# edantec/MPC_benchmark

Hardware: AMD Instinct MI355X
Metric: mpc_solves_per_sec (higher is better)
Workload: dtype f64

## Files before the change

### mpc_benchmark_amd/csrc/legs.h

```cpp
#pragma once
#include "mfma_blocks.h"
#include "solver_kernels.h"

#define LEG_BARRIER() asm volatile("s_waitcnt lgkmcnt(0)\n\ts_barrier" ::: "memory")

#define LEG_LAUNDER() do { asm volatile("" : "+v"(tid), "+v"(lane)); wv = __builtin_amdgcn_readfirstlane(tid >> 6); } while (0)

#define LK_THREADS 512
#define LK_U 20
#define LK_PT 13
#define LK_TILES 5

struct LkLds {
  int np, mp, nzp, lda, ldp, ldm, nb, nbm;
  int AB, PR, TM, ZN, vec, total_bytes;
  unsigned mg_nzp, mg_np, mg_mp;
};
static inline constexpr LkLds make_lk_lds(int n, int m) {
  LkLds s{};
  s.np = (n + 15) & ~15; s.mp = (m + 15) & ~15; s.nzp = s.np + s.mp; s.lda = s.nzp + 1; s.ldp = s.np + 1; s.ldm = s.mp + 1;
  s.nb = s.np / 16; s.nbm = s.mp / 16;
  s.mg_nzp = magic_div(s.nzp); s.mg_np = magic_div(s.np); s.mg_mp = magic_div(s.mp);
  int o = 0;
  auto take = [&](int cnt) { int r = o; o += (cnt + 1) & ~1; return r; };
  const int pr = s.np * s.ldp > s.mp * s.np + s.mp * s.ldm ? s.np * s.ldp : s.mp * s.np + s.mp * s.ldm;
  s.AB = take(s.np * s.lda); s.PR = take(pr); s.TM = take(6 * s.nzp + 6 * s.np + 40); s.ZN = take(16 * s.ldm); s.vec = take(s.mp + 3 * s.np + 80 + 8);
  s.total_bytes = o * 8;
  return s;
}

template <int MP, int FN = 0, int FM = 0>
DEV void leg_knot_body(const SolverArgs& a, const LkLds& Srt, const int b, const int kbeg, const int kend, const int prof_b, const int prof_k) {
  constexpr bool FX = FN > 0;
  constexpr LkLds SC_ = FX ? make_lk_lds(FN, FM) : LkLds{};
  LkLds S_ = Srt;
  if constexpr (FX) S_ = SC_;
  const LkLds& S = S_;
  constexpr int NAB = (80 * (80 + MP) + LK_THREADS - 1) / LK_THREADS, NK = (MP * 80 + LK_THREADS - 1) / LK_THREADS;
  constexpr int NMU = (MP * MP + LK_THREADS - 1) / LK_THREADS, NZN = (16 * MP + LK_THREADS - 1) / LK_THREADS;
  const Layout& L = a.L;
  int tid = threadIdx.x, lane = tid & 63;
  constexpr int nthr = LK_THREADS, nw = LK_THREADS / 64;
  int wv = __builtin_amdgcn_readfirstlane(tid >> 6);
  const InstState& st = a.inst[b];
  if (st.done || st.skip_step) return;
  const int n = FX ? FN : L.n, nz = FX ? FN + FM : L.nz, np = S.np, mp = S.mp, nzp = S.nzp, lda = S.lda, ldp = S.ldp, ldm = S.ldm, nb = S.nb, nbm = S.nbm;
  const double mud = st.mu * a.opt.dyn_al_scale;
  extern __shared__ __attribute__((aligned(16))) double sm[];
  double *AB = sm + S.AB, *PR = sm + S.PR, *ZN = sm + S.ZN, *vec = sm + S.vec;
  double *KM = PR, *PT = PR, *U1 = PR, *MU = PR + mp * np;
  double *TMP = sm + S.TM, *PT6 = TMP + 6 * nzp, *c6 = PT6 + 6 * np;
  double *kf = vec, *y0 = vec + mp, *z0 = y0 + np, *t6 = z0 + np, *g6 = t6 + 36, *mxs = g6 + 36;
  int* cnt = (int*)(mxs + np);
  long long tk0_ = clock64();
#define LK_PROF(slot) do { if (a.prof && k == prof_k && b == prof_b && tid == 0) { const long long t1_ = clock64(); a.prof[prof_b * 64 + 32 + (slot)] += (double)(t1_ - tk0_); tk0_ = t1_; } } while (0)

  double pab[NAB], pkm[NK], ptv[LK_PT], pmu[NMU], pzn[NZN], psm = 0.0, pact = 0.0;
  auto request_ab = [&](int k) {
    const double* kn = knot_ptr(a, b, k);
    const double* g = gain_ptr(a, b, k);
    const int m = (int)kn[L.oMISC + MISC_M], c = (int)kn[L.oMISC + MISC_NC];
#pragma unroll
    for (int u = 0; u < NAB; ++u) {
      const int idx = tid + u * nthr, i = qdiv(idx, S.mg_nzp), zp = (idx - qdiv(idx, S.mg_nzp) * nzp);
      const int z = (zp < n) ? zp : ((zp >= np && zp - np < m) ? n + zp - np : -1);
      pab[u] = (idx < np * nzp && i < n && z >= 0) ? kn[L.oAB + (size_t)i * nz + z] : 0.0;
    }
#pragma unroll
    for (int u = 0; u < NK; ++u) {
      const int idx = tid + u * nthr, l = qdiv(idx, S.mg_np), j = (idx - qdiv(idx, S.mg_np) * np);
      pkm[u] = (idx < mp * np && l < m && j < n) ? g[L.oK + l * n + j] : 0.0;
    }
    psm = (tid < mp) ? ((tid < m) ? g[L.ok + tid] : 0.0) : ((tid >= 64 && tid < 100) ? g[L.oT6 + tid - 64] : ((tid >= 128 && tid < 128 + n) ? g[L.omx + tid - 128] : 0.0));
    pact = (tid < c) ? kn[L.oACT + tid] : 0.0;
  };
  auto request_pt = [&](int k) {
    const double* g = gain_ptr(a, b, k);
#pragma unroll
    for (int u = 0; u < LK_PT; ++u) {
      const int idx = tid + u * nthr, i = qdiv(idx, S.mg_np), j = (idx - qdiv(idx, S.mg_np) * np);
      ptv[u] = (idx < np * np && i < n && j < n) ? g[L.oMx + i * n + j] : 0.0;
    }
  };
  auto request_mu = [&](int k) {
    const double* g = gain_ptr(a, b, k);
#pragma unroll
    for (int u = 0; u < NMU; ++u) { const int idx = tid + u * nthr; pmu[u] = (idx < mp * mp) ? g[L.oMu + idx] : 0.0; }
#pragma unroll
    for (int u = 0; u < NZN; ++u) { const int idx = tid + u * nthr; pzn[u] = (idx < 16 * mp) ? g[L.oZnu + idx] : 0.0; }
  };

  request_ab(kbeg);
  request_pt(kbeg);
  if (leg_of_knot(a, kbeg) + 1 < a.nlegs) request_mu(kbeg);
  for (int k = kbeg; k < kend; ++k) {
    const double* kn = knot_ptr(a, b, k);
    double* g = gain_ptr(a, b, k);
    const int m = (int)kn[L.oMISC + MISC_M];
    const bool par = leg_of_knot(a, k) + 1 < a.nlegs;
    const bool more = k + 1 < kend, par_next = more && leg_of_knot(a, k + 1) + 1 < a.nlegs;
    LEG_BARRIER();
    LEG_LAUNDER();
    if (a.prof) tk0_ = clock64();
#pragma unroll
    for (int u = 0; u < NAB; ++u) { const int idx = tid + u * nthr; if (idx < np * nzp) AB[(qdiv(idx, S.mg_nzp)) * lda + (idx - qdiv(idx, S.mg_nzp) * nzp)] = pab[u]; }
#pragma unroll
    for (int u = 0; u < NK; ++u) { const int idx = tid + u * nthr; if (idx < mp * np) KM[idx] = pkm[u]; }
    if (tid < mp) kf[tid] = psm;
    else if (tid >= 64 && tid < 100) t6[tid - 64] = psm;
    else if (tid >= 128 && tid < 128 + np) mxs[tid - 128] = psm;
    int ca = 0;
    if (par) {
      const unsigned long long act = __ballot(pact != 0.0);
      if (lane == 0) cnt[wv] = __popcll(act);
    }
    LEG_BARRIER();
    if (par) for (int w = 0; w < nw; ++w) ca += cnt[w];
    LEG_LAUNDER();
    if (more) request_ab(k + 1);
    LEG_LAUNDER();
    LK_PROF(0);
    for (int t = wv; t < nb * nb; t += nw) {
      const int ri = t / nb, cj = t % nb;
      double* At = AB + (ri * 16) * lda + cj * 16;
      d4_t acc = tile_load(At, lda, lane);
      mma_tile<false>(acc, AB + (ri * 16) * lda + np, lda, 1, KM + cj * 16, np, 1, mp, lane);
      tile_store(At, lda, acc, lane);
    }
    for (int i = wv; i < np; i += nw) {
      double s = (lane < m) ? AB[i * lda + np + lane] * kf[lane] : 0.0;
      s = wave_sum(s);
      if (lane == 0) y0[i] = s + mxs[i];
    }
    if (tid < 36) { const int i = tid / 6, j = tid % 6; double s = 0; for (int l = 0; l < 6; ++l) s += t6[i * 6 + l] * t6[j * 6 + l]; g6[tid] = s; }
    LEG_BARRIER();
    LEG_LAUNDER();
#pragma unroll
    for (int u = 0; u < LK_PT; ++u) { const int idx = tid + u * nthr; if (idx < np * np) PT[(qdiv(idx, S.mg_np)) * ldp + (idx - qdiv(idx, S.mg_np) * np)] = ptv[u]; }
    LEG_BARRIER();
    LEG_LAUNDER();
    if (more) request_pt(k + 1);
    LEG_LAUNDER();
    LK_PROF(1);
    const int nct = par ? nb + nbm : nb;
    d4_t res[LK_TILES];
#pragma unroll
    for (int sidx = 0; sidx < LK_TILES; ++sidx) {
      const int t = wv + sidx * nw;
      res[sidx] = d4_t{0, 0, 0, 0};
      if (t < nb * nct) mma_tile<false>(res[sidx], PT + ((t / nct) * 16) * ldp, ldp, 1, AB + (t % nct) * 16, lda, 1, np, lane);
    }
    for (int i = wv; i < n; i += nw) {
      double s = 0;
      for (int j = lane; j < n; j += 64) s += PT[i * ldp + j] * y0[j];
      s = wave_sum(s);
      if (lane == 0) z0[i] = y0[i] - mud * s;
    }
    LEG_BARRIER();
#pragma unroll
    for (int sidx = 0; sidx < LK_TILES; ++sidx) {
      const int t = wv + sidx * nw;
      if (t < nb * nct) {
        double* At = AB + ((t / nct) * 16) * lda + (t % nct) * 16;
        const int row = lane >> 4, col = lane & 15;
#pragma unroll
        for (int q = 0; q < 4; ++q) At[(row + 4 * q) * lda + col] -= mud * res[sidx][q];
      }
    }
    LEG_BARRIER();
    LK_PROF(2);
    for (int idx = tid; idx < 6 * nzp; idx += nthr) TMP[idx] = AB[(qdiv(idx, S.mg_nzp)) * lda + (idx - qdiv(idx, S.mg_nzp) * nzp)];
    if (par) for (int idx = tid; idx < np * 6; idx += nthr) {
      const int i = idx / 6, j = idx % 6;
      double s = 0;
      for (int l = 0; l < 6; ++l) s += PT[i * ldp + l] * t6[j * 6 + l];
      PT6[idx] = s;
    }
    LEG_BARRIER();
    for (int idx = tid; idx < 6 * nzp; idx += nthr) {
      const int i = qdiv(idx, S.mg_nzp), z = (idx - qdiv(idx, S.mg_nzp) * nzp);
      double s = 0;
      for (int l = 0; l < 6; ++l) s += t6[i * 6 + l] * TMP[l * nzp + z];
      AB[i * lda + z] = s;
    }
    if (par && tid < 36) {
      const int i = tid / 6, j = tid % 6;
      double s = 0;
      for (int l = 0; l < 6; ++l) s += t6[i * 6 + l] * PT6[l * 6 + j];
      c6[tid] = s;
    }
    LEG_BARRIER();
    for (int i = wv; i < n; i += nw)
      for (int j = lane; j < n; j += 64) g[L.oPhi + i * n + j] = AB[i * lda + j];
    for (int i = tid; i < n; i += nthr) {
      double s = z0[i];
      if (i < 6) { s = 0; for (int l = 0; l < 6; ++l) s += t6[i * 6 + l] * z0[l]; }
      g[L.ophi + i] = s;
    }
    LK_PROF(3);
    LEG_LAUNDER();
    if (par) {
#pragma unroll
      for (int u = 0; u < NMU; ++u) { const int idx = tid + u * nthr; if (idx < mp * mp) MU[(qdiv(idx, S.mg_mp)) * ldm + (idx - qdiv(idx, S.mg_mp) * mp)] = pmu[u]; }
#pragma unroll
      for (int u = 0; u < NZN; ++u) { const int idx = tid + u * nthr; if (idx < 16 * mp) ZN[(qdiv(idx, S.mg_mp)) * ldm + (idx - qdiv(idx, S.mg_mp) * mp)] = (qdiv(idx, S.mg_mp) < ca && ca <= 16) ? pzn[u] : 0.0; }
      LEG_BARRIER();
      LEG_LAUNDER();
      if (par_next) request_mu(k + 1);
      LEG_LAUNDER();
      LK_PROF(4);
      d4_t ures[2];
#pragma unroll
      for (int sidx = 0; sidx < 2; ++sidx) {
        const int t = wv + sidx * nw;
        ures[sidx] = d4_t{0, 0, 0, 0};
        if (t < nbm * nb) mma_tile<false>(ures[sidx], MU + ((t / nb) * 16) * ldm, ldm, 1, AB + ((t % nb) * 16) * lda + np, 1, lda, mp, lane);
      }
#ifdef LK_SUBPROF
      LK_PROF(7);
#endif
      if (ca <= 16) {
        for (int cj = wv; cj < nb; cj += nw) {
          d4_t acc = d4_t{0, 0, 0, 0};
          mma_tile<false>(acc, ZN, ldm, 1, AB + (cj * 16) * lda + np, 1, lda, mp, lane);
          const int col = cj * 16 + (lane & 15);
#pragma unroll
          for (int q = 0; q < 4; ++q) { const int row = (lane >> 4) + 4 * q; if (row < ca && col < n) g[L.oKnup + row * n + col] = -acc[q]; }
        }
      } else {
        for (int idx = tid; idx < ca * n; idx += nthr) {
          const int i = idx / n, j = idx % n;
          double s = 0;
          for (int l = 0; l < m; ++l) s += g[L.oZnu + i * mp + l] * AB[j * lda + np + l];
          g[L.oKnup + idx] = -s;
        }
      }
#ifdef LK_SUBPROF
      LK_PROF(8);
#endif
#pragma unroll
      for (int sidx = 0; sidx < 2; ++sidx) {
        const int t = wv + sidx * nw;
        if (t < nbm * nb) {
          const int ri = t / nb, cj = t % nb, col = cj * 16 + (lane & 15);
#pragma unroll
          for (int q = 0; q < 4; ++q) {
            const int row = ri * 16 + (lane >> 4) + 4 * q;
            U1[row * np + col] = ures[sidx][q];
            if (row < m && col < n) g[L.oKu + row * n + col] = -ures[sidx][q];
          }
        }
      }
#ifdef LK_SUBPROF
      LK_PROF(9);
#endif
      LEG_BARRIER();
      LK_PROF(5);
      for (int t = wv; t < nb * nb; t += nw) {
        const int ri = t / nb, cj = t % nb, col = cj * 16 + (lane & 15);
        double ptt[4];
#pragma unroll
        for (int q = 0; q < 4; ++q) {
          const int row = ri * 16 + (lane >> 4) + 4 * q;
          const bool in = row < n && col < n;
          ptt[q] = (in && row >= 6 && col >= 6) ? g[L.oMx + row * n + col] : 0.0;
        }
        d4_t acc = d4_t{0, 0, 0, 0};
        mma_tile<false>(acc, AB + (ri * 16) * lda + np, lda, 1, U1 + cj * 16, np, 1, mp, lane);
#pragma unroll
        for (int q = 0; q < 4; ++q) {
          const int row = ri * 16 + (lane >> 4) + 4 * q;
          if (row < n && col < n) {
            const double tt = (row < 6 && col < 6) ? g6[row * 6 + col] : (row == col ? 1.0 : 0.0);
            const double tp = (row < 6 && col < 6) ? c6[row * 6 + col] : (col < 6 ? PT6[row * 6 + col] : (row < 6 ? PT6[col * 6 + row] : ptt[q]));
            g[L.oGam + row * n + col] = -acc[q] - mud * (tt - mud * tp);
          }
        }
      }
      LK_PROF(6);
    } else if (par_next) request_mu(k + 1);
  }
}

template <int MP, int FN = 0, int FM = 0>
__global__ void __launch_bounds__(LK_THREADS) k_leg_knot(SolverArgs a, LkLds Srt, int chunk, int kmax) {
  const int kbeg = blockIdx.x * chunk, kend = (kbeg + chunk < kmax) ? kbeg + chunk : kmax;
  if (kbeg < kend) leg_knot_body<MP, FN, FM>(a, Srt, blockIdx.y, kbeg, kend, 1, 1);
}

struct LcLds { int np, ldp, nb; int LM, BA, BB, vec, total_bytes; unsigned mg_np, mg_ldp; };
static inline constexpr int lc_ld(int np) { int ld = np; while ((ld & 31) != 16) ++ld; return ld; }
static inline constexpr LcLds make_lc_lds(int n) {
  LcLds s{};
  s.np = (n + 15) & ~15; s.ldp = lc_ld(s.np); s.nb = s.np / 16;
  s.mg_np = magic_div(s.np); s.mg_ldp = magic_div(s.ldp);
  int o = 0;
  auto take = [&](int cnt) { int r = o; o += (cnt + 1) & ~1; return r; };
  s.LM = take(s.np * s.ldp); s.BA = take(s.np * s.ldp); s.BB = take(s.np * s.ldp); s.vec = take(3 * s.np + 16);
  s.total_bytes = o * 8;
  return s;
}
#define LC_TILES 4
#define LC_STILES 2

template <int FN = 0>
DEV void leg_condense_body(const SolverArgs& a, const LcLds& Srt, const int j, const int b) {
  constexpr bool FX = FN > 0;
  constexpr LcLds SC_ = FX ? make_lc_lds(FN) : LcLds{};
  LcLds S_ = Srt;
  if constexpr (FX) S_ = SC_;
  const LcLds& S = S_;
  const Layout& L = a.L;
  constexpr int nthr = LK_THREADS, nw = LK_THREADS / 64;
  int tid = threadIdx.x, lane = tid & 63, wv = __builtin_amdgcn_readfirstlane(tid >> 6);
  const InstState& st = a.inst[b];
  if (st.done || st.skip_step) return;
  const int n = FX ? FN : L.n, np = S.np, ldp = S.ldp, nb = S.nb;
  const int ks = leg_start(a, j), ke = leg_start(a, j + 1) - 1;
  extern __shared__ __attribute__((aligned(16))) double sm[];
  double *LM = sm + S.LM, *BA = sm + S.BA, *BB = sm + S.BB, *sg = sm + S.vec, *phi = sg + np;
  for (int idx = tid; idx < np * ldp; idx += nthr) { const int i = qdiv(idx, S.mg_ldp), c0 = (idx - qdiv(idx, S.mg_ldp) * ldp); LM[idx] = (i == c0 && i < n) ? 1.0 : 0.0; }
  for (int i = tid; i < np; i += nthr) sg[i] = 0.0;
  d4_t sacc[LC_STILES];
  int tri[LC_STILES], tcj[LC_STILES];
#pragma unroll
  for (int sidx = 0; sidx < LC_STILES; ++sidx) {
    sacc[sidx] = d4_t{0, 0, 0, 0};
    int ri = 0, rem = wv + sidx * nw;
    while (rem > ri) { rem -= ri + 1; ++ri; }
    tri[sidx] = ri; tcj[sidx] = rem;
  }
  const int nst = nb * (nb + 1) / 2;
  double pa[LK_PT], pb[LK_PT], pphi;
  auto prefetch = [&](int kk) {
    const double* gk = gain_ptr(a, b, kk);
#pragma unroll
    for (int u = 0; u < LK_PT; ++u) {
      const int idx = tid + u * nthr, i = qdiv(idx, S.mg_np), c0 = (idx - qdiv(idx, S.mg_np) * np);
      const bool ok = idx < np * np && i < n && c0 < n;
      const int src = ok ? i * n + c0 : 0;
      pa[u] = gk[L.oPhi + src] * (ok ? 1.0 : 0.0);
      pb[u] = gk[L.oGam + src] * (ok ? 1.0 : 0.0);
    }
    pphi = gk[L.ophi + (tid < n ? tid : 0)];
  };
  prefetch(ke);
  long long tc0_ = clock64();
#define LC_PROF(slot) do { if (a.prof && j == 0 && b == 2 && tid == 0) { const long long t1_ = clock64(); a.prof[128 + 32 + (slot)] += (double)(t1_ - tc0_); tc0_ = t1_; } } while (0)
  for (int k = ke; k >= ks; --k) {
    LEG_LAUNDER();
#pragma unroll
    for (int u = 0; u < LK_PT; ++u) {
      const int idx = tid + u * nthr;
      if (idx < np * np) { BA[(qdiv(idx, S.mg_np)) * ldp + (idx - qdiv(idx, S.mg_np) * np)] = pa[u]; BB[(qdiv(idx, S.mg_np)) * ldp + (idx - qdiv(idx, S.mg_np) * np)] = pb[u]; }
    }
    if (tid < np) phi[tid] = (tid < n) ? pphi : 0.0;
    LEG_BARRIER();
    LC_PROF(0);
    LEG_LAUNDER();
    if (k > ks) prefetch(k - 1);
    LEG_LAUNDER();
    d4_t lres[LC_TILES], zres[LC_TILES];
#pragma unroll
    for (int sidx = 0; sidx < LC_TILES; ++sidx) {
      const int t = wv + sidx * nw;
      lres[sidx] = d4_t{0, 0, 0, 0}; zres[sidx] = d4_t{0, 0, 0, 0};
      if (t < nb * nb)
        mma_tile_2a(lres[sidx], zres[sidx], BA + (t / nb) * 16, 1, ldp, BB + (t / nb) * 16, 1, ldp, LM + (t % nb) * 16, ldp, 1, np, lane);
    }
    LC_PROF(1);
    {
      const int ts = tid - (nthr - 128);
      if (ts >= 0 && ts < n) {
        double s = 0;
#pragma unroll 16
        for (int l = 0; l < np; ++l) s += LM[l * ldp + ts] * phi[l];
        sg[ts] += s;
      }
    }
    LC_PROF(2);
    LEG_BARRIER();
    LC_PROF(3);
    LEG_LAUNDER();
#pragma unroll
    for (int sidx = 0; sidx < LC_TILES; ++sidx) {
      const int t = wv + sidx * nw;
      if (t < nb * nb) tile_store(BB + ((t / nb) * 16) * ldp + (t % nb) * 16, ldp, zres[sidx], lane);
    }
    LEG_BARRIER();
    LC_PROF(4);
    LEG_LAUNDER();
#pragma unroll
    for (int sidx = 0; sidx < LC_STILES; ++sidx)
      if (wv + sidx * nw < nst) mma_tile<false>(sacc[sidx], LM + tri[sidx] * 16, 1, ldp, BB + tcj[sidx] * 16, ldp, 1, np, lane);
    LC_PROF(5);
    LEG_BARRIER();
    LC_PROF(6);
    LEG_LAUNDER();
    double* gk = gain_ptr(a, b, k);
#pragma unroll
    for (int sidx = 0; sidx < LC_TILES; ++sidx) {
      const int t = wv + sidx * nw;
      if (t < nb * nb) {
        const int ri = t / nb, cj = t % nb, col = cj * 16 + (lane & 15);
        tile_store(LM + (ri * 16) * ldp + cj * 16, ldp, lres[sidx], lane);
#pragma unroll
        for (int q = 0; q < 4; ++q) { const int row = ri * 16 + (lane >> 4) + 4 * q; if (row < n && col < n) gk[L.oLm + row * n + col] = lres[sidx][q]; }
// ... 499 lines not shown
```

### mpc_benchmark_amd/csrc/mpc_hip.hip

```cpp
#include <hip/hip_runtime.h>
#include <mutex>
#include <map>
#include <cmath>
#include <cstdio>
#include <cstdlib>
#include <cstring>
#include <limits>
#include <stdexcept>
#include <string>
#include <utility>
#include <vector>

#include "eval_multibody_host.h"
#include "eval_reuse_kernels.h"
#include "eval_vector.h"
#include "riccati_mfma.h"
#include "closed_loop.h"
#include "legs.h"
#include "legs_tree.h"
#include "pipeline_glue.h"
#include "pipeline_ikid_glue.h"
#include "pipeline_contacts.h"
#include "pipeline_fd_glue.h"
#include "sim_record.h"
// ... 117 lines not shown
  bool spec_rec_valid = false, spec_next_pending = false, spec_next_now = false;
  int cycles_since_run = 0;
  int khead = 0;
  int* d_spec = nullptr;
  double* d_fext = nullptr;
  int only_knot = -1;
  bool appended_changed = false;
  bool appended_any = false;
  bool walk_on = false, walk_force_all = false;
  std::vector<uint8_t> walk_poisoned;
  mpc_walk_config walk{};
  double* d_walk_state = nullptr;
  double *d_walk_cmd = nullptr, *d_poses_cmd = nullptr;
  bool walk_cmd_on = false, poses_cmd_on = false;
  bool poses_on = false;
  mpc_walk_poses_config poses{};
  double *d_poses_state = nullptr, *d_poses_samples = nullptr, *d_poses_x = nullptr;
  size_t poses_x_cap = 0;
  int since_change = 1 << 20;
  bool refine_now = false;
  SimPlant plant;
  std::vector<uint8_t> slot_dirty;
  bool dirty_all = false;
  bool spec_skip_pass = false;
  unsigned long long dirty_now[MPC_DIRTY_WORDS] = {};
  static constexpr int PATCH_RING = 4;
  char* patch_pin[PATCH_RING] = {};
  size_t patch_cap[PATCH_RING] = {};
  hipEvent_t patch_ev[PATCH_RING] = {};
  int patch_next = 0;
  char* d_patch = nullptr;
  size_t d_patch_cap = 0;
  double* h_xnext[2] = {nullptr, nullptr};
  std::vector<double> leg_mu;
  static constexpr int ASYNC_DEPTH = 2;
  InstState* h_status[ASYNC_DEPTH] = {nullptr, nullptr};
  hipEvent_t status_ev[ASYNC_DEPTH] = {nullptr, nullptr};
  int async_head = 0, async_pending = 0;
  static constexpr int STAGE_RING = 8;
  char* stage_pin[STAGE_RING] = {};
  hipEvent_t stage_ev[STAGE_RING] = {};
  int stage_next = 0;
  RicLds ric{};
  int ric_fixed = 0;
  ClLds cl{};
  bool use_mfma_riccati = false;
  LkLds lk{};
  LcLds lc{};
  LxLds lx{};
  bool legs_ok = false;
  bool env_chain = false, env_plain = false, env_reject_failed = false;
  int env_tree_sweeps = 0, env_trace = -1;
  int env_tail_knots = -1, cu_count = 0;
  int tail_last = 0, tail_sweeps_last = 0;
  long long tail_fused = 0, tail_separate = 0;
  long long leg_passes_multi = 0, leg_passes_single = 0;
  int leg_tail_knots(int J) const {
    if (J < 2 || env_tail_knots == 0) return 0;
    const int last = L.N - (int)((long long)(J - 1) * L.N / J);
    if (env_tail_knots > 0) return env_tail_knots < last ? env_tail_knots : last;
    if ((long long)J * L.B > cu_count || (long long)L.N * L.B <= cu_count) return 0;
    const int t = 21 * (L.N / J) / 25;
    return t < last ? t : last;
  }
  int env_apply_chunk = -1;
  bool env_duals_plain = false;
  int apply_chunk_last = 0;
  long long apply_chunked = 0, apply_single = 0;
  long long duals_staged = 0, duals_plain = 0;
  int leg_apply_chunk(int J) const {
    int C;
    if (env_apply_chunk > 0) C = env_apply_chunk;
    else C = (long long)L.N * L.B <= cu_count ? 1 : 5;
    return C < 1 ? 1 : (C > LEG_APPLY_MAX_CHUNK ? LEG_APPLY_MAX_CHUNK : C);
  }
  double* d_legbuf = nullptr;
  double* d_treebuf = nullptr;
  int leg_cap = 0;
  TreeDesc tree{};
  bool use_tree() const {
    return eff_legs() >= 3 && d_treebuf != nullptr && !env_chain;
  }
  bool leg_guess_valid = false;
  int leg_guess_now = 0;
  int eff_legs() const {
    if (!legs_ok) return 1;
    int J = opt.riccati_legs;
    if (J > MPC_MAX_LEGS) J = MPC_MAX_LEGS;
    if (J > L.N) J = L.N;
    return J < 1 ? 1 : J;
  }
  struct ProfSlot {
    const char* name;
    std::vector<std::pair<hipEvent_t, hipEvent_t>> ev;
    size_t used = 0;
  };
  bool profiling = false;
  unsigned prof_mask = ~0u;
  std::vector<ProfSlot> prof;

  template <class F> void timed(int slot, const char* name, F&& launch) {
    if (!profiling || !((prof_mask >> slot) & 1u) || pass_is_corrector) { launch(); return; }
    if ((int)prof.size() <= slot) prof.resize(slot + 1);
    ProfSlot& p = prof[slot];
    p.name = name;
    if (p.used == p.ev.size()) {
      hipEvent_t e0, e1;
      HIP_OK(hipEventCreate(&e0));
      HIP_OK(hipEventCreate(&e1));
      p.ev.emplace_back(e0, e1);
    }
    HIP_OK(hipEventRecord(p.ev[p.used].first, stream));
    launch();
    HIP_OK(hipEventRecord(p.ev[p.used].second, stream));
    p.used++;
// ... 22 lines not shown
    a.reuse_same = (a.reuse_on && reuse_same_now) ? 1 : 0;
    a.spec_knot = a.spec_on ? d_spec_knot : nullptr; a.spec_next = (a.reuse_on && spec_next_now) ? 1 : 0;
    for (int w = 0; w < MPC_DIRTY_WORDS; ++w) a.dirty[w] = a.reuse_on ? dirty_now[w] : 0ull;
    a.only_knot = only_knot;
    a.corrector_on = corrector_armed() ? 1 : 0;
    a.reject_failed = env_reject_failed ? 1 : 0;
    a.tree_pivoted = getenv("MPC_HIP_TREE_PIVOTED") ? 1 : 0;
    a.nlegs = eff_legs(); a.leg_cap = leg_cap; a.legbuf = d_legbuf; a.treebuf = d_treebuf; a.leg_guess = leg_guess_now;
    a.knots = d_knots; a.gains = d_gains; a.work = d_work; a.trial_phi = d_trial_phi; a.inst = d_inst; a.all_done = d_all_done; a.prof = phase_timers ? d_prof : nullptr;
    return a;
  }
  size_t riccati_lds() const {
    return ((size_t)L.n * L.n + (size_t)L.m * L.m + (size_t)L.sc_cap * L.sc_cap) * sizeof(double) + ((size_t)L.c + 4) * sizeof(int);
  }
};

static void copy_sync(mpc_solver* s, void* dst, const void* src, size_t bytes, hipMemcpyKind kind) {
  HIP_OK(hipMemcpyAsync(dst, src, bytes, kind, s->stream));
  HIP_OK(hipStreamSynchronize(s->stream));
}

static void ensure_leg_capacity(mpc_solver* s, int legs) {
  const Layout& L = s->L;
  int need = legs < 1 ? 1 : legs;
  if (need >= 3 && need < 4) need = 4;
  if (need <= s->leg_cap) return;
  HIP_OK(hipStreamSynchronize(s->stream));
  auto regrow = [&](double*& p, size_t count) {
    if (p) HIP_OK(hipFree(p));
    p = nullptr;
    HIP_OK(hipMalloc((void**)&p, (count ? count : 1) * sizeof(double)));
    HIP_OK(hipMemsetAsync(p, 0, (count ? count : 1) * sizeof(double), s->stream));
  };
  const size_t B = L.B;
  regrow(s->d_work, B * need * (size_t)L.work_stride);
  if (s->legs_ok) {
    regrow(s->d_legbuf, B * (size_t)(need > 1 ? need - 1 : 1) * L.leg_stride);
    regrow(s->d_treebuf, B * (size_t)need * L.tree_stride);
  }
  s->leg_cap = need;
  s->leg_guess_valid = false;
  HIP_OK(hipStreamSynchronize(s->stream));
}

static void create_impl(mpc_solver* s, const mpc_dims& d) {
  s->dims = d;
  { const char* e;
    e = getenv("MPC_LEGS_CHAIN"); s->env_chain = e && atoi(e) > 0;
    e = getenv("MPC_LEGS_PLAIN"); s->env_plain = e && atoi(e) > 0;
    e = getenv("MPC_HIP_REJECT_FAILED"); s->env_reject_failed = e && atoi(e) > 0;
    e = getenv("MPC_TREE_SWEEPS"); s->env_tree_sweeps = e ? atoi(e) : 0;
    e = getenv("MPC_HIP_TRACE"); s->env_trace = e ? atoi(e) : -1;
    e = getenv("MPC_LEG_TAIL_KNOTS"); s->env_tail_knots = e ? (atoi(e) > 0 ? atoi(e) : 0) : -1;
    e = getenv("MPC_LEG_APPLY_CHUNK"); s->env_apply_chunk = (e && atoi(e) > 0) ? atoi(e) : -1;
    e = getenv("MPC_DUALS_PLAIN"); s->env_duals_plain = e && atoi(e) > 0; }
  HIP_OK(hipSetDevice(d.device));
  HIP_OK(hipDeviceGetAttribute(&s->cu_count, hipDeviceAttributeMultiprocessorCount, d.device));
  { const char* e = getenv("MPC_LEG_TAIL_CUS"); if (e && atoi(e) > 0) s->cu_count = atoi(e); }
  {
    static int created = 0;
    const char* pe = getenv("MPC_HIP_STREAM_PRIO");
    if (pe && atoi(pe) > 0) {
      int lo = 0, hi = 0;
      HIP_OK(hipDeviceGetStreamPriorityRange(&lo, &hi));
      const int levels = lo - hi + 1;
      const int prio = hi + (created++ % levels);
      HIP_OK(hipStreamCreateWithPriority(&s->stream, hipStreamNonBlocking, prio));
      if (atoi(pe) > 1) fprintf(stderr, "[mpc] stream priority %d (range %d..%d)\n", prio, hi, lo);
    } else {
      HIP_OK(hipStreamCreateWithFlags(&s->stream, hipStreamNonBlocking));
    }
  }
  Layout& L = s->L;
  L.N = d.horizon; L.B = d.batch; L.space = d.space; L.nx = d.nx; L.n = d.ndx; L.m = d.nu; L.c = d.nc_max > 0 ? d.nc_max : 1;
  L.nj = 0;
  L.max_stage_ints = d.max_stage_ints; L.max_stage_doubles = d.max_stage_doubles;
  L.n_alpha = 8;
  make_layout(L);
  Layout& T = s->LT;
  T = L;
  {
    int o = 0;
    auto take = [&](int cnt) { int r = o; o += align2(cnt); return r; };
    T.oCV = take(L.c); T.oCT = take(L.c); T.oLO = take(L.c); T.oHI = take(L.c); T.oDT = take(L.c); T.oACT = take(L.c);
    T.oF = take(L.n); T.oMISC = take(MISC_COUNT);
    T.oH = T.oG = T.oAB = T.oE6 = T.oT6k = T.oD12 = T.oCD = T.oXD = T.oWR = T.oXN = 0;
    T.knot_stride = o;
  }
  if (s->riccati_lds() > 160 * 1024) throw std::runtime_error("problem dimensions exceed the LDS budget of the Riccati kernel");
  const size_t B = d.batch, N1 = d.horizon + 1, N = d.horizon;
  s->d_stage_desc = s->alloc<int32_t>(N1 * L.max_stage_ints);
  s->d_stage_params = s->alloc<double>(N1 * L.max_stage_doubles);
  s->d_xs = s->alloc<double>(B * N1 * L.nx); s->d_us = s->alloc<double>(B * N * L.m + 1);
  s->d_xs_alt = s->alloc<double>(B * N1 * L.nx); s->d_us_alt = s->alloc<double>(B * N * L.m + 1);
  s->d_vs = s->alloc<double>(B * N1 * L.c); s->d_lams = s->alloc<double>(B * (N1 + 1) * L.n);
  s->d_vs_e = s->alloc<double>(B * N1 * L.c); s->d_lams_e = s->alloc<double>(B * (N1 + 1) * L.n);
  s->d_x0 = s->alloc<double>(B * L.nx);
  s->d_dxs = s->alloc<double>(B * (N1 + 1) * L.n); s->d_dus = s->alloc<double>(B * N * L.m + 1);
  s->d_dvs = s->alloc<double>(B * N1 * L.c); s->d_dlams = s->alloc<double>(B * (N1 + 1) * L.n); s->d_abdz = s->alloc<double>(B * N1 * L.n);
  s->d_knots = s->alloc<double>(B * N1 * L.knot_stride);
  s->d_tknots = s->alloc<double>(B * L.n_alpha * N1 * T.knot_stride);
  s->d_gains = s->alloc<double>(B * N1 * L.gain_stride);
  s->d_trial_phi = s->alloc<double>(B * L.n_alpha * N1);
  s->d_inst = s->alloc<InstState>(B);
  s->d_all_done = s->alloc<int>(4);
  s->d_spec = s->alloc<int>(B);
// ... 265 lines not shown
    launch_eval_multibody(s->stream, a, s->LT, (trial && !with_derivs) ? s->d_tknots : s->d_knots, s->d_mbwork, s->mb_work_stride, trial, cand0, ncand, with_derivs, s->contact_dyn);
  }
  HIP_OK(hipGetLastError());
}

static void launch_pass(mpc_solver* s) {
  const Layout& L = s->L;
  if (s->pass_in_run > 0 && s->tick_reuse && s->opt.max_iters <= 4) {
    s->reuse_this_pass = true; s->reuse_same_now = true;
    for (int w = 0; w < MPC_DIRTY_WORDS; ++w) s->dirty_now[w] = 0ull;
  }
  SolverArgs a = s->args();
  if (a.spec_next) hipLaunchKernelGGL(k_copy_spec, dim3(32, L.B), dim3(256), 0, s->stream, a);
  s->timed(0, "k_eval_stage", [&] { launch_eval(s, false); });
  if (a.reuse_on) hipLaunchKernelGGL(k_reproject, dim3(L.N + 1, L.B), dim3(256), 0, s->stream, a);
  s->reuse_this_pass = false; s->reuse_same_now = false;
  s->spec_next_now = false;
  s->timed(1, "k_lagrangian", [&] { hipLaunchKernelGGL(k_lagrangian, dim3(L.N + 1, L.B), dim3(64), 0, s->stream, a); });
  s->timed(2, "k_decide", [&] { hipLaunchKernelGGL(k_decide, dim3(L.B), dim3(128), 0, s->stream, a); });
  a.abdz = nullptr;
  const int J = a.nlegs;
  const bool plain = s->env_plain;
  const bool tree = s->use_tree();
  if (tree && s->tree.J != J) s->tree = make_tree_desc(J);
  int sweeps = (J > 1 && !plain && !s->leg_guess_valid) ? (tree ? s->tree.nlev + 1 : 2) : 1;
  if (tree && !plain && s->env_tree_sweeps > sweeps) sweeps = s->env_tree_sweeps;
  const int tail = s->leg_tail_knots(J);
  s->tail_last = tail; s->tail_sweeps_last = sweeps;
  if (J > 1) { if (sweeps > 1) s->leg_passes_multi++; else s->leg_passes_single++; }
  for (int sweep = 0; sweep < sweeps; ++sweep) {
  s->leg_guess_now = (J > 1 && !plain && (s->leg_guess_valid || sweep > 0)) ? 1 : 0;
  a = s->args();
  a.abdz = nullptr;
  s->timed(3, "k_riccati_backward", [&] {
    if (J > 1) {
      if (s->ric.np == 16 && s->ric.mp == 16 && L.c <= RIC_SMALL_THREADS)
        hipLaunchKernelGGL(HIP_KERNEL_NAME(k_riccati_mfma<RIC_SMALL_THREADS, 16, false, true>), dim3(L.B * J), dim3(RIC_SMALL_THREADS), s->ric.total_bytes, s->stream, a, s->ric);
#define X(ID, FN, FM, GF, ST, NPV, MPV) else if (s->ric_fixed == ID) hipLaunchKernelGGL(HIP_KERNEL_NAME(k_riccati_mfma<RIC_THREADS, 80, true, true, FN, FM, GF, ST>), dim3(L.B * J), dim3(RIC_THREADS), s->ric.total_bytes, s->stream, a, s->ric);
      MPC_FIXED_MODELS(X)
#undef X
      else if (s->ric.sq) hipLaunchKernelGGL(HIP_KERNEL_NAME(k_riccati_mfma<RIC_THREADS, 80, true, true>), dim3(L.B * J), dim3(RIC_THREADS), s->ric.total_bytes, s->stream, a, s->ric);
      else hipLaunchKernelGGL(HIP_KERNEL_NAME(k_riccati_mfma<RIC_THREADS, 80, false, true>), dim3(L.B * J), dim3(RIC_THREADS), s->ric.total_bytes, s->stream, a, s->ric);
    }
    else if (s->use_mfma_riccati && s->ric.np == 16 && s->ric.mp == 16 && L.c <= RIC_SMALL_THREADS)
      hipLaunchKernelGGL(HIP_KERNEL_NAME(k_riccati_mfma<RIC_SMALL_THREADS, 16>), dim3(L.B), dim3(RIC_SMALL_THREADS), s->ric.total_bytes, s->stream, a, s->ric);
    else if (s->use_mfma_riccati && s->ric.sq && s->ric.np <= 80) hipLaunchKernelGGL(HIP_KERNEL_NAME(k_riccati_mfma<RIC_THREADS, 80, true>), dim3(L.B), dim3(RIC_THREADS), s->ric.total_bytes, s->stream, a, s->ric);
    else if (s->use_mfma_riccati && s->ric.sq) hipLaunchKernelGGL(HIP_KERNEL_NAME(k_riccati_mfma<RIC_THREADS, 96, true>), dim3(L.B), dim3(RIC_THREADS), s->ric.total_bytes, s->stream, a, s->ric);
    else if (s->use_mfma_riccati && s->ric.np <= 80) hipLaunchKernelGGL(HIP_KERNEL_NAME(k_riccati_mfma<RIC_THREADS, 80>), dim3(L.B), dim3(RIC_THREADS), s->ric.total_bytes, s->stream, a, s->ric);
    else if (s->use_mfma_riccati) hipLaunchKernelGGL(HIP_KERNEL_NAME(k_riccati_mfma<RIC_THREADS, 96>), dim3(L.B), dim3(RIC_THREADS), s->ric.total_bytes, s->stream, a, s->ric);
    else hipLaunchKernelGGL(k_riccati_backward, dim3(L.B), dim3(256), s->riccati_lds(), s->stream, a);
  });
  if (J > 1) {
    s->timed(12, "k_closed_loop", [&] {
      static const int chunk_env = getenv("MPC_LEG_KNOT_CHUNK") ? atoi(getenv("MPC_LEG_KNOT_CHUNK")) : 0;
      const int chunk = chunk_env > 0 ? chunk_env : 1;
      const int kmax = L.N - tail;
      const dim3 grid((kmax + chunk - 1) / chunk, L.B);
      if (false) {}
#define X(ID, FN, FM, GF, ST, NPV, MPV) else if (s->ric_fixed == ID) hipLaunchKernelGGL((k_leg_knot<MPV, FN, FM>), grid, dim3(LK_THREADS), s->lk.total_bytes, s->stream, a, s->lk, chunk, kmax);
      MPC_FIXED_MODELS(X)
#undef X
      else if (s->lk.mp <= 16) hipLaunchKernelGGL(k_leg_knot<16>, grid, dim3(LK_THREADS), s->lk.total_bytes, s->stream, a, s->lk, chunk, kmax);
      else if (s->lk.mp <= 32) hipLaunchKernelGGL(k_leg_knot<32>, grid, dim3(LK_THREADS), s->lk.total_bytes, s->stream, a, s->lk, chunk, kmax);
      else hipLaunchKernelGGL(k_leg_knot<48>, grid, dim3(LK_THREADS), s->lk.total_bytes, s->stream, a, s->lk, chunk, kmax);
    });
    if (tail > 0) s->timed(13, "k_leg_condense", [&] {
      const int lds = s->lc.total_bytes > s->lk.total_bytes ? s->lc.total_bytes : s->lk.total_bytes;
      const dim3 grid(J, L.B);
      s->tail_fused++;
      if (false) {}
#define X(ID, FN, FM, GF, ST, NPV, MPV) else if (s->ric_fixed == ID) hipLaunchKernelGGL((k_leg_condense_tail<MPV, FN, FM>), grid, dim3(LK_THREADS), lds, s->stream, a, s->lc, s->lk, tail);
      MPC_FIXED_MODELS(X)
#undef X
      else if (s->lk.mp <= 16) hipLaunchKernelGGL(k_leg_condense_tail<16>, grid, dim3(LK_THREADS), lds, s->stream, a, s->lc, s->lk, tail);
      else if (s->lk.mp <= 32) hipLaunchKernelGGL(k_leg_condense_tail<32>, grid, dim3(LK_THREADS), lds, s->stream, a, s->lc, s->lk, tail);
      else hipLaunchKernelGGL(k_leg_condense_tail<48>, grid, dim3(LK_THREADS), lds, s->stream, a, s->lc, s->lk, tail);
    });
    else s->timed(13, "k_leg_condense", [&] {
      s->tail_separate++;
      if (false) {}
#define X(ID, FN, FM, GF, ST, NPV, MPV) else if (s->ric_fixed == ID) hipLaunchKernelGGL(k_leg_condense<FN>, dim3(J - 1, L.B), dim3(LK_THREADS), s->lc.total_bytes, s->stream, a, s->lc);
      MPC_FIXED_MODELS(X)
#undef X
      else hipLaunchKernelGGL(k_leg_condense<0>, dim3(J - 1, L.B), dim3(LK_THREADS), s->lc.total_bytes, s->stream, a, s->lc);
    });
    if (tree) s->timed(14, "k_leg_consensus", [&] {
      const TreeDesc& T = s->tree;
#define MPC_TREE_LAUNCH(NPV) do { \
        for (int lev = 0; lev < T.nlev; ++lev) hipLaunchKernelGGL(k_leg_compose<NPV>, dim3(T.lev_cnt[lev] + 1, L.B, 2), dim3(LCMP_THREADS), s->lx.total_bytes, s->stream, a, s->lx, T, lev); } while (0)
      if (false) {
#define X(ID, FN, FM, GF, ST, NPV, MPV) } else if (s->ric_fixed == ID) { for (int lev = 0; lev < T.nlev; ++lev) hipLaunchKernelGGL((k_leg_compose<NPV, FN, FM>), dim3(T.lev_cnt[lev] + 1, L.B, 2), dim3(LCMP_THREADS), s->lx.total_bytes, s->stream, a, s->lx, T, lev);
      MPC_FIXED_MODELS(X)
#undef X
      } else switch (s->lx.np) {
        case 16: MPC_TREE_LAUNCH(16); break;
        case 32: MPC_TREE_LAUNCH(32); break;
        case 48: MPC_TREE_LAUNCH(48); break;
        case 64: MPC_TREE_LAUNCH(64); break;
        default: MPC_TREE_LAUNCH(80); break;
      }
#undef MPC_TREE_LAUNCH
    });
    if (tree) s->timed(16, "k_leg_tree_down", [&] {
      const TreeDesc& T = s->tree;
      if (false) {
#define X(ID, FN, FM, GF, ST, NPV, MPV) } else if (s->ric_fixed == ID) { for (int lev = T.nlev - 1; lev >= 0; --lev) hipLaunchKernelGGL((k_leg_tree_down<NPV, FN, FM>), dim3(T.lev_cnt[lev] + (lev == T.nlev - 1 ? 1 : 0), L.B), dim3(LK_THREADS), s->lx.total_bytes, s->stream, a, s->lx, T, lev);
      MPC_FIXED_MODELS(X)
#undef X
// ... 966 lines not shown
```

Before: 12330.

## Use row-mapped 16-byte vector loads for fixed-model leg knot and condense staging

For compile-time fixed models, the global-to-LDS staging of A|B, K, P, Mu, Znu, Phi and Gamma switches from flat index decomposition with magic division to a row-per-wave mapping with double2 loads. It also adds fast paths that skip bounds checks on interior tiles when writing Ku and Gamma, and replaces the per-knot leg lookup with a comparison against the last leg's start. The default tail-knot fraction is retuned and the chunk env read moves into solver init. The goal is fewer global transactions and less index arithmetic, at the cost of more registers and alignment assumptions enforced by static_asserts.

After: 12630, median of 6. 1.02x the previous value.

```diff
diff --git a/mpc_benchmark_amd/csrc/legs.h b/mpc_benchmark_amd/csrc/legs.h
--- a/mpc_benchmark_amd/csrc/legs.h
+++ b/mpc_benchmark_amd/csrc/legs.h
@@ -10,6 +10,9 @@
 #define LK_U 20
 #define LK_PT 13
 #define LK_TILES 5
+
+DEV double2 leg_ld2(const double* p) { return *(const double2*)p; }
+DEV void leg_st2(double* p, double2 v) { *(double2*)p = v; }
 
 struct LkLds {
   int np, mp, nzp, lda, ldp, ldm, nb, nbm;
@@ -56,10 +59,40 @@
 #define LK_PROF(slot) do { if (a.prof && k == prof_k && b == prof_b && tid == 0) { const long long t1_ = clock64(); a.prof[prof_b * 64 + 32 + (slot)] += (double)(t1_ - tk0_); tk0_ = t1_; } } while (0)
 
   double pab[NAB], pkm[NK], ptv[LK_PT], pmu[NMU], pzn[NZN], psm = 0.0, pact = 0.0;
+  static_assert(!FX || (FN % 2 == 0 && FM % 2 == 0), "row-mapped moves: column pairs must not straddle the A | B boundary and must be 16-byte aligned");
+  constexpr int XNP = FX ? SC_.np : 16, XMP = FX ? SC_.mp : 16, XRW = XNP / (LK_THREADS / 64), XRK = XMP / (LK_THREADS / 64);
+  constexpr int XML = XMP / 2, XMR = 64 / XML, XQM = (XMP + 8 * XMR - 1) / (8 * XMR), XQZ = (16 + 8 * XMR - 1) / (8 * XMR);
+  static_assert(!FX || (XNP + XMP <= 128 && XML <= 64 && XMP % XMR == 0 && 16 % XMR == 0), "row-mapped moves: a row of [A B] is at most 64 column pairs, whole groups of Mu / Znu rows");
+  double2 rab[XRW], rkm[XRK], rpt[XRW], rmu[XQM], rzn[XQZ];
   auto request_ab = [&](int k) {
     const double* kn = knot_ptr(a, b, k);
     const double* g = gain_ptr(a, b, k);
     const int m = (int)kn[L.oMISC + MISC_M], c = (int)kn[L.oMISC + MISC_NC];
+    if constexpr (FX) {
+      const int zp = 2 * lane;
+      const bool isa = zp < FN;
+      const double* src = kn + L.oAB + wv * (FN + FM) + (isa ? zp : zp - (XNP - FN));
+      const bool ld = isa || (zp >= XNP && zp - XNP < m);
+#pragma unroll
+      for (int r = 0; r < XRW; ++r) rab[r] = double2{0.0, 0.0};
+      if (ld) {
+#pragma unroll
+        for (int r = 0; r < XRW; ++r) if (8 * r + 7 < FN || wv + 8 * r < FN) rab[r] = leg_ld2(src + 8 * r * (FN + FM));
+      }
+      const double* ksrc = g + L.oK + wv * FN + zp;
+#pragma unroll
+      for (int r = 0; r < XRK; ++r) rkm[r] = double2{0.0, 0.0};
+      if (isa) {
+#pragma unroll
+        for (int r = 0; r < XRK; ++r) if (wv + 8 * r < m) rkm[r] = leg_ld2(ksrc + 8 * r * FN);
+      }
+      psm = 0.0;
+      if (wv == 0) { if (lane < m) psm = g[L.ok + lane]; }
+      else if (wv == 1) { if (lane < 36) psm = g[L.oT6 + lane]; }
+      else if (wv < 4) { if (tid - 128 < FN) psm = g[L.omx + tid - 128]; }
+      pact = (tid < c) ? kn[L.oACT + tid] : 0.0;
+      return;
+    }
 #pragma unroll
     for (int u = 0; u < NAB; ++u) {
       const int idx = tid + u * nthr, i = qdiv(idx, S.mg_nzp), zp = (idx - qdiv(idx, S.mg_nzp) * nzp);
@@ -76,6 +109,16 @@
   };
   auto request_pt = [&](int k) {
     const double* g = gain_ptr(a, b, k);
+    if constexpr (FX) {
+      const double* src = g + L.oMx + wv * FN + 2 * lane;
+#pragma unroll
+      for (int r = 0; r < XRW; ++r) rpt[r] = double2{0.0, 0.0};
+      if (2 * lane < FN) {
+#pragma unroll
+        for (int r = 0; r < XRW; ++r) if (8 * r + 7 < FN || wv + 8 * r < FN) rpt[r] = leg_ld2(src + 8 * r * FN);
+      }
+      return;
+    }
 #pragma unroll
     for (int u = 0; u < LK_PT; ++u) {
       const int idx = tid + u * nthr, i = qdiv(idx, S.mg_np), j = (idx - qdiv(idx, S.mg_np) * np);
@@ -84,24 +127,52 @@
   };
   auto request_mu = [&](int k) {
     const double* g = gain_ptr(a, b, k);
+    if constexpr (FX) {
+      const int sub = lane / XML, off = (wv * XMR + sub) * XMP + 2 * (lane - sub * XML);
+      const bool on = lane < XMR * XML;
+#pragma unroll
+      for (int q = 0; q < XQM; ++q) { rmu[q] = double2{0.0, 0.0}; if ((wv + 8 * q) * XMR < XMP && on) rmu[q] = leg_ld2(g + L.oMu + off + 8 * q * XMR * XMP); }
+#pragma unroll
+      for (int q = 0; q < XQZ; ++q) { rzn[q] = double2{0.0, 0.0}; if ((wv + 8 * q) * XMR < 16 && on) rzn[q] = leg_ld2(g + L.oZnu + off + 8 * q * XMR * XMP); }
+      return;
+    }
 #pragma unroll
     for (int u = 0; u < NMU; ++u) { const int idx = tid + u * nthr; pmu[u] = (idx < mp * mp) ? g[L.oMu + idx] : 0.0; }
 #pragma unroll
     for (int u = 0; u < NZN; ++u) { const int idx = tid + u * nthr; pzn[u] = (idx < 16 * mp) ? g[L.oZnu + idx] : 0.0; }
   };
 
+  const int klast = FX ? leg_start(a, a.nlegs - 1) : 0;
+  auto parametric = [&](int k) { if constexpr (FX) return k < klast; else return leg_of_knot(a, k) + 1 < a.nlegs; };
   request_ab(kbeg);
   request_pt(kbeg);
-  if (leg_of_knot(a, kbeg) + 1 < a.nlegs) request_mu(kbeg);
+  if (parametric(kbeg)) request_mu(kbeg);
   for (int k = kbeg; k < kend; ++k) {
     const double* kn = knot_ptr(a, b, k);
     double* g = gain_ptr(a, b, k);
     const int m = (int)kn[L.oMISC + MISC_M];
-    const bool par = leg_of_knot(a, k) + 1 < a.nlegs;
-    const bool more = k + 1 < kend, par_next = more && leg_of_knot(a, k + 1) + 1 < a.nlegs;
+    const bool par = parametric(k);
+    const bool more = k + 1 < kend, par_next = more && parametric(k + 1);
     LEG_BARRIER();
     LEG_LAUNDER();
     if (a.prof) tk0_ = clock64();
+    if constexpr (FX) {
+      const int zp = 2 * lane;
+      if (zp < XNP + XMP) {
+        const bool hi = zp < XNP || zp + 1 - XNP < m;
+        double* d = AB + wv * lda + zp;
+#pragma unroll
+        for (int r = 0; r < XRW; ++r) { d[8 * r * lda] = rab[r].x; d[8 * r * lda + 1] = hi ? rab[r].y : 0.0; }
+      }
+      if (zp < XNP) {
+        double* d = KM + wv * XNP + zp;
+#pragma unroll
+        for (int r = 0; r < XRK; ++r) leg_st2(d + 8 * r * XNP, rkm[r]);
+      }
+      if (wv == 0) { if (lane < XMP) kf[lane] = psm; }
+      else if (wv == 1) { if (lane < 36) t6[lane] = psm; }
+      else if (wv < 4) { if (tid - 128 < XNP) mxs[tid - 128] = psm; }
+    } else {
 #pragma unroll
     for (int u = 0; u < NAB; ++u) { const int idx = tid + u * nthr; if (idx < np * nzp) AB[(qdiv(idx, S.mg_nzp)) * lda + (idx - qdiv(idx, S.mg_nzp) * nzp)] = pab[u]; }
 #pragma unroll
@@ -109,6 +180,7 @@
     if (tid < mp) kf[tid] = psm;
     else if (tid >= 64 && tid < 100) t6[tid - 64] = psm;
     else if (tid >= 128 && tid < 128 + np) mxs[tid - 128] = psm;
+    }
     int ca = 0;
     if (par) {
       const unsigned long long act = __ballot(pact != 0.0);
@@ -135,8 +207,16 @@
     if (tid < 36) { const int i = tid / 6, j = tid % 6; double s = 0; for (int l = 0; l < 6; ++l) s += t6[i * 6 + l] * t6[j * 6 + l]; g6[tid] = s; }
     LEG_BARRIER();
     LEG_LAUNDER();
+    if constexpr (FX) {
+      if (2 * lane < XNP) {
+        double* d = PT + wv * ldp + 2 * lane;
+#pragma unroll
+        for (int r = 0; r < XRW; ++r) { d[8 * r * ldp] = rpt[r].x; d[8 * r * ldp + 1] = rpt[r].y; }
+      }
+    } else {
 #pragma unroll
     for (int u = 0; u < LK_PT; ++u) { const int idx = tid + u * nthr; if (idx < np * np) PT[(qdiv(idx, S.mg_np)) * ldp + (idx - qdiv(idx, S.mg_np) * np)] = ptv[u]; }
+    }
     LEG_BARRIER();
     LEG_LAUNDER();
     if (more) request_pt(k + 1);
@@ -200,10 +280,22 @@
     LK_PROF(3);
     LEG_LAUNDER();
     if (par) {
+      if constexpr (FX) {
+        const int sub = lane / XML, off = (wv * XMR + sub) * ldm + 2 * (lane - sub * XML);
+        const bool on = lane < XMR * XML;
+#pragma unroll
+        for (int q = 0; q < XQM; ++q) if ((wv + 8 * q) * XMR < XMP && on) { double* d = MU + off + 8 * q * XMR * ldm; d[0] = rmu[q].x; d[1] = rmu[q].y; }
+#pragma unroll
+        for (int q = 0; q < XQZ; ++q) if ((wv + 8 * q) * XMR < 16 && on) {
+          const bool live = (wv + 8 * q) * XMR + sub < ca && ca <= 16;
+          double* d = ZN + off + 8 * q * XMR * ldm; d[0] = live ? rzn[q].x : 0.0; d[1] = live ? rzn[q].y : 0.0;
+        }
+      } else {
 #pragma unroll
       for (int u = 0; u < NMU; ++u) { const int idx = tid + u * nthr; if (idx < mp * mp) MU[(qdiv(idx, S.mg_mp)) * ldm + (idx - qdiv(idx, S.mg_mp) * mp)] = pmu[u]; }
 #pragma unroll
       for (int u = 0; u < NZN; ++u) { const int idx = tid + u * nthr; if (idx < 16 * mp) ZN[(qdiv(idx, S.mg_mp)) * ldm + (idx - qdiv(idx, S.mg_mp) * mp)] = (qdiv(idx, S.mg_mp) < ca && ca <= 16) ? pzn[u] : 0.0; }
+      }
       LEG_BARRIER();
       LEG_LAUNDER();
       if (par_next) request_mu(k + 1);
@@ -243,11 +335,20 @@
         const int t = wv + sidx * nw;
         if (t < nbm * nb) {
           const int ri = t / nb, cj = t % nb, col = cj * 16 + (lane & 15);
+          if (FX && ri * 16 + 15 < m && cj + 1 < nb) {
+#pragma unroll
+            for (int q = 0; q < 4; ++q) {
+              const int row = ri * 16 + (lane >> 4) + 4 * q;
+              U1[row * np + col] = ures[sidx][q];
+              g[L.oKu + row * n + col] = -ures[sidx][q];
+            }
+          } else {
 #pragma unroll
           for (int q = 0; q < 4; ++q) {
             const int row = ri * 16 + (lane >> 4) + 4 * q;
             U1[row * np + col] = ures[sidx][q];
             if (row < m && col < n) g[L.oKu + row * n + col] = -ures[sidx][q];
+          }
           }
         }
       }
@@ -259,6 +360,20 @@
       for (int t = wv; t < nb * nb; t += nw) {
         const int ri = t / nb, cj = t % nb, col = cj * 16 + (lane & 15);
         double ptt[4];
+        if (FX && ri > 0 && cj > 0 && ri + 1 < nb && cj + 1 < nb) {
+#pragma unroll
+          for (int q = 0; q < 4; ++q) ptt[q] = g[L.oMx + (ri * 16 + (lane >> 4) + 4 * q) * n + col];
+          d4_t acc = d4_t{0, 0, 0, 0};
+          mma_tile<false>(acc, AB + (ri * 16) * lda + np, lda, 1, U1 + cj * 16, np, 1, mp, lane);
+#pragma unroll
+          for (int q = 0; q < 4; ++q) {
+            const int row = ri * 16 + (lane >> 4) + 4 * q;
+            const double tt = row == col ? 1.0 : 0.0;
+            const double tp = ptt[q];
+            g[L.oGam + row * n + col] = -acc[q] - mud * (tt - mud * tp);
+          }
+          continue;
+        }
 #pragma unroll
         for (int q = 0; q < 4; ++q) {
           const int row = ri * 16 + (lane >> 4) + 4 * q;
@@ -332,8 +447,22 @@
   }
   const int nst = nb * (nb + 1) / 2;
   double pa[LK_PT], pb[LK_PT], pphi;
+  static_assert(!FX || FN % 2 == 0, "row-mapped moves: 16-byte column pairs");
+  constexpr int XNP = FX ? SC_.np : 16, XRW = XNP / (LK_THREADS / 64);
+  double2 ra[XRW], rb[XRW];
   auto prefetch = [&](int kk) {
     const double* gk = gain_ptr(a, b, kk);
+    if constexpr (FX) {
+      const double* src = gk + wv * FN + 2 * lane;
+#pragma unroll
+      for (int r = 0; r < XRW; ++r) { ra[r] = double2{0.0, 0.0}; rb[r] = double2{0.0, 0.0}; }
+      if (2 * lane < FN) {
+#pragma unroll
+        for (int r = 0; r < XRW; ++r) if (8 * r + 7 < FN || wv + 8 * r < FN) { ra[r] = leg_ld2(src + L.oPhi + 8 * r * FN); rb[r] = leg_ld2(src + L.oGam + 8 * r * FN); }
+      }
+      pphi = gk[L.ophi + (tid < n ? tid : 0)];
+      return;
+    }
 #pragma unroll
     for (int u = 0; u < LK_PT; ++u) {
       const int idx = tid + u * nthr, i = qdiv(idx, S.mg_np), c0 = (idx - qdiv(idx, S.mg_np) * np);
@@ -349,10 +478,18 @@
 #define LC_PROF(slot) do { if (a.prof && j == 0 && b == 2 && tid == 0) { const long long t1_ = clock64(); a.prof[128 + 32 + (slot)] += (double)(t1_ - tc0_); tc0_ = t1_; } } while (0)
   for (int k = ke; k >= ks; --k) {
     LEG_LAUNDER();
+    if constexpr (FX) {
+      if (2 * lane < XNP) {
+        const int off = wv * ldp + 2 * lane;
+#pragma unroll
+        for (int r = 0; r < XRW; ++r) { leg_st2(BA + off + 8 * r * ldp, ra[r]); leg_st2(BB + off + 8 * r * ldp, rb[r]); }
+      }
+    } else {
 #pragma unroll
     for (int u = 0; u < LK_PT; ++u) {
       const int idx = tid + u * nthr;
       if (idx < np * np) { BA[(qdiv(idx, S.mg_np)) * ldp + (idx - qdiv(idx, S.mg_np) * np)] = pa[u]; BB[(qdiv(idx, S.mg_np)) * ldp + (idx - qdiv(idx, S.mg_np) * np)] = pb[u]; }
+    }
     }
     if (tid < np) phi[tid] = (tid < n) ? pphi : 0.0;
     LEG_BARRIER();
diff --git a/mpc_benchmark_amd/csrc/mpc_hip.hip b/mpc_benchmark_amd/csrc/mpc_hip.hip
--- a/mpc_benchmark_amd/csrc/mpc_hip.hip
+++ b/mpc_benchmark_amd/csrc/mpc_hip.hip
@@ -193,6 +193,7 @@
   bool env_chain = false, env_plain = false, env_reject_failed = false;
   int env_tree_sweeps = 0, env_trace = -1;
   int env_tail_knots = -1, cu_count = 0;
+  int env_knot_chunk = 0;
   int tail_last = 0, tail_sweeps_last = 0;
   long long tail_fused = 0, tail_separate = 0;
   long long leg_passes_multi = 0, leg_passes_single = 0;
@@ -201,7 +202,7 @@
     const int last = L.N - (int)((long long)(J - 1) * L.N / J);
     if (env_tail_knots > 0) return env_tail_knots < last ? env_tail_knots : last;
     if ((long long)J * L.B > cu_count || (long long)L.N * L.B <= cu_count) return 0;
-    const int t = 21 * (L.N / J) / 25;
+    const int t = 4 * (L.N / J) / 5;
     return t < last ? t : last;
   }
   int env_apply_chunk = -1;
@@ -330,6 +331,7 @@
     e = getenv("MPC_TREE_SWEEPS"); s->env_tree_sweeps = e ? atoi(e) : 0;
     e = getenv("MPC_HIP_TRACE"); s->env_trace = e ? atoi(e) : -1;
     e = getenv("MPC_LEG_TAIL_KNOTS"); s->env_tail_knots = e ? (atoi(e) > 0 ? atoi(e) : 0) : -1;
+    e = getenv("MPC_LEG_KNOT_CHUNK"); s->env_knot_chunk = (e && atoi(e) > 0) ? atoi(e) : 0;
     e = getenv("MPC_LEG_APPLY_CHUNK"); s->env_apply_chunk = (e && atoi(e) > 0) ? atoi(e) : -1;
     e = getenv("MPC_DUALS_PLAIN"); s->env_duals_plain = e && atoi(e) > 0; }
   HIP_OK(hipSetDevice(d.device));
@@ -701,8 +703,7 @@
   });
   if (J > 1) {
     s->timed(12, "k_closed_loop", [&] {
-      static const int chunk_env = getenv("MPC_LEG_KNOT_CHUNK") ? atoi(getenv("MPC_LEG_KNOT_CHUNK")) : 0;
-      const int chunk = chunk_env > 0 ? chunk_env : 1;
+      const int chunk = s->env_knot_chunk > 0 ? s->env_knot_chunk : 1;
       const int kmax = L.N - tail;
       const dim3 grid((kmax + chunk - 1) / chunk, L.B);
       if (false) {}
```
